# lucas-t-t/FACT-CLIP

Hardware: AMD Instinct MI355X
Metric: frames/sec FACT_CLIP fwd+bwd, T=4096 D=2048 Nact=32, at 1/2/4/8 GPUs (higher is better)
Workload: dtype fp32; 1 GPU; FACT_CLIP HAViD-holdout dims, seg10 synthetic, T=4096; model=FACT_CLIP, T=4096, D=2048, Nact=32, C=75, videos_per_rank=2, global_batch=2, seq_len=4096, parallelism=dp1, weights=fixed (no optimizer update in the timed steps)

## Files before the change

fact-clip_amd/csrc/capi.cpp:

```cpp
#include <algorithm>
#include <atomic>
#include <tuple>
#include <map>
#include <mutex>
#include <cmath>
#include <cstdlib>
#include <cstring>
#include <mutex>
#include <vector>

#include "fx_common.h"
#include "ops.h"

namespace fx {

static thread_local std::string g_last_error;
void set_error(const std::string& msg) { g_last_error = msg; }

namespace {
struct ProfState {
  int max_events = 0;
  std::vector<hipEvent_t> ev;
  std::vector<double> flops, bytes;
  std::vector<int> launches;
// ... 414 lines not shown
  long long d = p->dil0 > 0 ? p->dil0 : 1;
  const int f = p->dil_factor > 0 ? p->dil_factor : 2;
  for (int k = 0; k < i; ++k) d *= f;
  return (int)d;
}

bool mstcn_defer_ok(const fx_mstcn_params* p, const fx_mstcn_grads* g) {
  if (!knobs().mstcn_defer) return false;
  const int NL = p->num_layers;
  for (int i = 0; i < NL; ++i)
    if (!g->w_dil[i] || !g->b_dil[i] || !g->w_pw[i] || !g->b_pw[i]) return false;
  auto uniform = [&](float* const* v) {
    for (int i = 2; i < NL; ++i)
      if (v[i] - v[i - 1] != v[1] - v[0]) return false;
    return true;
  };
  return uniform(g->w_dil) && uniform(g->b_dil) && uniform(g->w_pw) && uniform(g->b_pw);
}

struct Seqs {
  int T, nvid;
  const int* off;
  int rows() const { return off ? off[nvid] : T * nvid; }
  int start(int v) const { return off ? off[v] : v * T; }
  int len(int v) const { return off ? off[v + 1] - off[v] : T; }
};

int check_seqs(const Seqs& q) {
  FX_REQUIRE(q.nvid >= 1, "frame branch: nvid >= 1");
  if (!q.off) {
    FX_REQUIRE(q.T >= 1, "frame branch: T >= 1");
    return FX_OK;
  }
  FX_REQUIRE(q.nvid <= 16 && q.off[0] == 0, "frame branch: ragged offsets start at 0, <= 16 videos");
  for (int v = 0; v < q.nvid; ++v) FX_REQUIRE(q.off[v + 1] > q.off[v], "frame branch: empty video");
  return FX_OK;
}

fx_operand conv_operand(const float* h, long long ld, int cin, int dil, int dir, const Seqs& q, bool trans) {
  fx_operand o = trans ? op_cols(h, ld) : op_rows(h, ld);
  o.conv_taps = 3;
  o.conv_cin = cin;
  o.conv_dil = dil;
  o.conv_dir = dir;
  if (q.off) {
    o.seq_off = q.off;
    o.nseq = q.nvid;
  } else {
    o.seq_len = q.T;
  }
  return o;
}

template <typename Fn>
int per_video(const Seqs& q, Fn fn) {
  if (!q.off) return fn(0, q.rows(), q);
  for (int v = 0; v < q.nvid; ++v) FX_TRY(fn(q.start(v), q.len(v), Seqs{q.len(v), 1, nullptr}));
  return FX_OK;
}

}
}

using namespace fx;

extern "C" {

int fx_version(void) { return FX_ABI_VERSION; }

}

namespace fx {
const Knobs& knobs() {
  static Knobs k;
  static std::once_flag once;
  std::call_once(once, [] {
    auto env = [](const char* n) -> const char* { return std::getenv(n); };
    if (const char* p = env("FX_GEMM_PATH")) k.gemm_path = std::string(p) == "tiled" ? 1 : std::string(p) == "direct" ? 2 : 0;
    if (const char* p = env("FX_GEMM_W8")) k.gemm_w8 = p[0] == '1';
    if (const char* p = env("FX_GEMM_WIDE")) k.gemm_wide = p[0] == '1' ? 1 : 0;
    if (const char* p = env("FX_GEMM_XCDPLANES")) k.gemm_xcd_planes = p[0] != '0';
    if (const char* p = env("FX_GEMM_GROUP")) k.gemm_group = p[0] != '0';
    if (const char* p = env("FX_GEMM_KTAIL")) k.gemm_ktail = p[0] != '0';
    if (const char* p = env("FX_DEC_TOK")) k.dec_tok = p[0] != '0';
    if (const char* p = env("FX_TOK_SPIN")) k.tok_spin = std::max(0, std::atoi(p));
    if (const char* p = env("FX_SIDE_STREAM")) k.side_stream = p[0] != '0';
    if (const char* p = env("FX_MSTCN_DEFER")) k.mstcn_defer = p[0] != '0';
    if (const char* p = env("FX_GEMM_ROWPERM")) k.gemm_row_perm = p[0] != '0';
    if (const char* p = env("FX_GEMM_GROUPM")) k.gemm_group_m = p[0] != '0';
    if (const char* p = env("FX_GEMM_PERSIST")) k.gemm_persist = p[0] != '0';
    if (const char* p = env("FX_FRL_XCD")) k.frl_xcd = std::atoi(p);
    if (const char* p = env("FX_FRL_PAIR")) k.frl_pair = p[0] != '0';
    if (const char* p = env("FX_FRL_MIN_FILL")) k.frl_min_fill = std::atoi(p);
    if (const char* p = env("FX_AUX_STREAM")) k.aux_stream = p[0] != '0';
    if (const char* p = env("FX_GRU_POLL2")) k.gru_poll2 = p[0] != '0';
    if (const char* p = env("FX_GRU_STORE_WAVE")) k.gru_store_wave = std::max(0, std::min(2, std::atoi(p)));
    if (const char* p = env("FX_TATTN_RR")) k.tattn_rr = p[0] != '0';
    if (const char* p = env("FX_X2Y_A2F_DW")) k.x2y_a2f_dw = p[0] != '0';
    if (const char* p = env("FX_TATTN_FOLD")) k.tattn_fold = p[0] != '0';
    if (const char* p = env("FX_X2Y_FUSED")) k.x2y_fused = p[0] != '0';
    if (const char* p = env("FX_X2Y_F2A_BWD")) k.x2y_f2a_bwd = std::atoi(p);
    if (const char* p = env("FX_X2Y_F2A_ONE")) k.x2y_f2a_one = p[0] != '0';
  });
  return k;
}
}

extern "C" {
const char* fx_last_error(void) { return g_last_error.c_str(); }

int fx_dropout(const float* x, long long ldx, int rows, int cols, long long idx_ld, long long idx_col0, float p,
               unsigned long long seed, float* y, long long ldy, void* stream) {
  FX_REQUIRE(x && y && rows >= 0 && cols >= 0, "dropout: bad arguments");
  return launch_dropout(x, ldx, rows, cols, idx_ld, idx_col0, p, seed, y, ldy, (hipStream_t)stream);
}

long long fx_struct_size(int which) {
  switch (which) {
    case 0: return (long long)sizeof(fx_gemm_desc);
    case 1: return (long long)sizeof(fx_decoder_params);
    case 2: return (long long)sizeof(fx_mstcn_params);
    case 3: return (long long)sizeof(fx_loss_term);
    case 4: return (long long)sizeof(fx_video_attn);
    case 5: return (long long)sizeof(fx_mstcn2_params);
    default: return -1;
  }
}

int fx_gemm(const fx_gemm_desc* desc, void* stream) {
  FX_REQUIRE(desc, "fx_gemm: null descriptor");
  const bool conv = desc->a.conv_taps && !desc->a.trans;
  if (conv) prof_begin(0, (hipStream_t)stream);
  const int st = launch_gemm(*desc, (hipStream_t)stream);
  if (conv) prof_end(0, (hipStream_t)stream, 2.0 * desc->M * desc->N * desc->K * desc->batch, 0.0);
  return st;
}

long long fx_gemm_workspace_floats(const fx_gemm_desc* desc) { return desc ? gemm_workspace_floats(*desc) : 0; }

int fx_linear_fwd(const float* x, long long ldx, const float* pos, long long ldpos, int pos_cols, int M, int K,
                  const float* w, long long ldw, const float* b, float* y, long long ldy, int N, int relu,
                  void* stream) {
  return linear_fwd(x, ldx, M, K, w, b, y, ldy, N, relu, (hipStream_t)stream, ldw, pos, ldpos, pos_cols);
}

long long fx_linear_bwd_workspace_floats(int M, int K, int N) {
  return (long long)M * N + split_ws(M, K, N) + dwdb_ws(M, K, N) + colsum_workspace_floats(M, N);
}

int fx_linear_bwd(const float* dy, long long lddy, const float* x, long long ldx, const float* w, long long ldw,
                  const float* relu_out, long long ld_relu, int M, int K, int N, float* dx, long long lddx,
                  float* dw, long long lddw, float* db, int accumulate_dx, int accumulate_w, float* workspace,
                  void* stream) {
  hipStream_t s = (hipStream_t)stream;
  FX_REQUIRE(workspace || (!relu_out && split_ws(M, K, N) == 0 && dwdb_ws(M, K, N) == 0 && !(db && !dw)),
             "fx_linear_bwd: workspace required");
  float* wz = workspace;
  float* wsx = wz + (long long)M * N;
  float* wsw = wsx + split_ws(M, K, N);
  float* wsc = wsw + dwdb_ws(M, K, N);
  const float* g = dy;
  long long ldg = lddy;
  if (relu_out) {
    FX_TRY(relu_bwd(dy, lddy, relu_out, ld_relu, M, N, wz, N, s));
    g = wz;
    ldg = N;
// ... 1490 lines not shown
```

fact-clip_amd/csrc/fx_common.h:

```cpp
#pragma once
#include <hip/hip_runtime.h>
#include <hip/hip_ext.h>
#include <cstdint>
#include <cstdio>
#include <string>

#include "../../include/factmx.h"

namespace fx {

void set_error(const std::string& msg);

#define FX_CHECK_HIP(expr)                                                        \
  do {                                                                            \
    hipError_t _e = (expr);                                                       \
    if (_e != hipSuccess) {                                                       \
      ::fx::set_error(std::string("HIP error ") + hipGetErrorString(_e) + " at " + \
                      __FILE__ + ":" + std::to_string(__LINE__));                 \
      return FX_ERR_HIP;                                                          \
    }                                                                             \
  } while (0)

#define FX_REQUIRE(cond, msg)                 \
  do {                                        \
    if (!(cond)) {                            \
      ::fx::set_error(std::string(msg));      \
      return FX_ERR_SHAPE;                    \
    }                                         \
  } while (0)

#define FX_TRY(expr)                 \
  do {                               \
    int _s = (expr);                 \
    if (_s != FX_OK) return _s;      \
  } while (0)

inline int cdiv(long long a, long long b) { return (int)((a + b - 1) / b); }
inline long long al64(long long n) { return (n + 63) & ~63LL; }

int launch_gemm(const fx_gemm_desc& d, hipStream_t s);
int launch_gemm_group(const fx_gemm_desc* d, int n, hipStream_t s);

struct WsBound {
  WsBound(const float* base, long long floats);
  ~WsBound();
  const float* prev_lo;
  const float* prev_hi;
};
hipStream_t side_fork(hipStream_t s, int event);
int side_join_into(hipStream_t s);
hipStream_t aux_fork(hipStream_t s);
int aux_join_into(hipStream_t s, hipStream_t a);
int defer_split(int rows);
long long gemm_workspace_floats(const fx_gemm_desc& d);

fx_operand op_rows(const float* p, long long ld);
fx_operand op_cols(const float* p, long long ld);
fx_gemm_desc gemm_desc(int M, int N, int K, fx_operand a, fx_operand b, float* c, long long ldc);

int launch_colsum_batched(const float* x, long long ld, long long x_bs, int M, int N, int nb, float* out,
                          long long out_bs, int accumulate, float* ws, hipStream_t s);
int launch_colsum(const float* x, long long ld, int M, int N, float* out, int accumulate,
                  float* ws, hipStream_t s);

constexpr long long kArrivalCounters = 1 << 16;
unsigned* arrival_counters(hipStream_t s);

__host__ __device__ inline unsigned fx_drop_bits(unsigned long long seed, unsigned long long idx) {
  unsigned long long z = seed + (idx + 1ull) * 0x9E3779B97F4A7C15ull;
  z = (z ^ (z >> 30)) * 0xBF58476D1CE4E5B9ull;
  z = (z ^ (z >> 27)) * 0x94D049BB133111EBull;
  z ^= z >> 31;
  return (unsigned)(z >> 32);
}
inline unsigned fx_drop_thresh(float p) {
  const double t = (double)p * 4294967296.0;
  return t >= 4294967295.0 ? 4294967295u : (unsigned)t;
}
inline unsigned long long fx_drop_subseed(unsigned long long seed, int i) {
  return seed + 0xD1B54A32D192ED03ull * (unsigned long long)(i + 1);
}
int launch_dropout(const float* x, long long ldx, int rows, int cols, long long idx_ld, long long idx_col0, float p,
                   unsigned long long seed, float* y, long long ldy, hipStream_t s);

struct Knobs {
  int gemm_path = 0;
  bool gemm_w8 = true;
  int gemm_wide = -1;
  bool gemm_xcd_planes = true;
  bool gemm_persist = true;
  bool gemm_group_m = true;
  bool gemm_row_perm = true;
  bool frl_pair = true;
  int frl_min_fill = 80;
  bool aux_stream = true;
  bool x2y_a2f_dw = true;
  bool tattn_fold = true;
  bool tattn_rr = true;
  bool gru_poll2 = true;
  int gru_store_wave = 2;
  int frl_xcd = 2;
  bool gemm_group = true;
  bool gemm_ktail = true;
  bool dec_tok = true;
  int tok_spin = 0;
  bool side_stream = true;
  bool mstcn_defer = true;
  bool x2y_fused = true;
  bool x2y_f2a_one = true;
  int x2y_f2a_bwd = 2;
};
const Knobs& knobs();

void prof_begin(int kind, hipStream_t s);
void prof_end(int kind, hipStream_t s, double flops, double bytes, int launches = 1);
extern thread_local int g_prof_open;
bool prof_kernel_events(hipStream_t s, hipEvent_t* e0, hipEvent_t* e1);

template <typename... Args, typename F = void (*)(Args...)>
inline void fx_launch(F kernel, const dim3& grid, const dim3& block, std::uint32_t shm, hipStream_t s, Args... args) {
  hipEvent_t e0, e1;
  if (g_prof_open >= 0 && prof_kernel_events(s, &e0, &e1))
    hipExtLaunchKernelGGL(kernel, grid, block, shm, s, e0, e1, 0u, args...);
  else
    hipLaunchKernelGGL(kernel, grid, block, shm, s, args...);
}

unsigned tok_spin_max();
unsigned x2y_spin_max();
int coresident_blocks(const void* kernel, int threads, size_t lds);

}
```

fact-clip_amd/csrc/gemm_f32.hip:

```cpp
#include <algorithm>
#include <atomic>
#include <cstdio>
#include <cstdlib>
#include <map>
#include <mutex>
#include <string>
#include <utility>
#include <vector>

#include "fx_common.h"

namespace fx {
namespace {

constexpr int BM = 64, BN = 64, BK = 64, NTHREADS = 256;
constexpr int RS = 68;
constexpr int CS = 65;
constexpr int IMG = BM * RS;
constexpr int NSLOT = 3;
typedef float f32x16 __attribute__((ext_vector_type(16)));

constexpr int kMaxSeq = 16;

enum Kind { ROWS = 0, ROWS_CONV = 1, ROWS_GEN = 2, COLS = 3, COLS_CONV = 4, ROWS_CAT = 5, COLS_CONVR = 6, COLS_KT = 7 };
// ... 1617 lines not shown
      if constexpr (AK == COLS_KT) {
        if (!fast) break;
        fx_launch((gemm_f32_kernel<AK, COLS_KT, true>), grid, dim3(NTHREADS), 0, s, g);
        return FX_OK;
      }
      break;
    case ROWS_GEN:
    case ROWS_CAT: launch_t<AK, ROWS_GEN>(grid, s, g, false); return FX_OK;
    default: break;
  }
  set_error("gemm: unsupported B operand kind");
  return FX_ERR_UNSUPPORTED;
}

int launch_tiled(int ak, int bk, dim3 grid, hipStream_t s, const GemmDev& g) {
  const bool fast = g.a_vec && g.b_vec && ((g.K % BK) == 0 || ak == COLS_KT) && ak != ROWS_GEN && bk != ROWS_GEN;
  switch (ak) {
    case ROWS: return launch_b<ROWS>(bk, grid, s, g, fast);
    case ROWS_CONV: return launch_b<ROWS_CONV>(bk, grid, s, g, fast);
    case ROWS_GEN: return launch_b<ROWS_GEN>(bk, grid, s, g, false);
    case ROWS_CAT: return launch_b<ROWS_CAT>(bk, grid, s, g, fast);
    case COLS: return launch_b<COLS>(bk, grid, s, g, fast);
    case COLS_KT: return launch_b<COLS_KT>(bk, grid, s, g, fast);
    default: break;
  }
  set_error("gemm: unsupported A operand kind");
  return FX_ERR_UNSUPPORTED;
}

template <int AK>
int launch_direct_b(int bk, dim3 grid, dim3 block, hipStream_t s, const GemmDev& g) {
  switch (bk) {
    case ROWS: fx_launch((gemm_direct_kernel<AK, ROWS>), grid, block, 0, s, g); return FX_OK;
    case COLS: fx_launch((gemm_direct_kernel<AK, COLS>), grid, block, 0, s, g); return FX_OK;
    default: break;
  }
  set_error("gemm(direct): unsupported B operand kind");
  return FX_ERR_UNSUPPORTED;
}

int launch_direct(int ak, int bk, dim3 grid, dim3 block, hipStream_t s, const GemmDev& g) {
  switch (ak) {
    case ROWS: return launch_direct_b<ROWS>(bk, grid, block, s, g);
    case ROWS_GEN:
    case ROWS_CAT: return launch_direct_b<ROWS_GEN>(bk, grid, block, s, g);
    case COLS: return launch_direct_b<COLS>(bk, grid, block, s, g);
    default: break;
  }
  set_error("gemm(direct): unsupported A operand kind");
  return FX_ERR_UNSUPPORTED;
}

bool use_direct(const fx_gemm_desc& d, int ak, int bk) {
  const int force = knobs().gemm_path;
  auto fits = [&](const fx_operand& o, int kind, int R) {
    const double k = (double)d.K + 2 * DMAXW * DCH + 64, ld = (double)o.ld;
    const double bytes = kind == ROWS ? ((double)R * ld + k) * 4 : kind == COLS ? (k * ld + R) * 4 : 0;
    return bytes < 4294967296.0;
  };
  const bool ok = d.K > 0 && (ak == ROWS || ak == ROWS_GEN || ak == ROWS_CAT || ak == COLS) && (bk == ROWS || bk == COLS) &&
                  fits(d.a, ak, d.M) && fits(d.b, bk, d.N);
  if (!ok || force == 1) return false;
  if (force == 2) return true;
  const int lim = (ak == ROWS_GEN || ak == ROWS_CAT) ? 32 : 64;
  if (d.M <= lim || d.N <= lim || d.K <= 64 || (d.K <= 512 && d.K % 64 != 0)) return true;
  const long long t32 = (long long)cdiv(d.M, 32) * cdiv(d.N, 32) * d.batch;
  return (ak == ROWS || ak == COLS) && t32 <= 512 && d.K <= 2048;
}

bool wide8() {
  return knobs().gemm_w8;
}

bool use_wide(const GemmDev& g, int ak, int bk, int batch) {
  const int force = knobs().gemm_wide;
  const bool fast = g.a_vec && g.b_vec && ((g.K % BK) == 0 || ak == COLS_KT);
  const bool ok = fast && (ak == ROWS || ak == ROWS_CONV || ak == ROWS_CAT || ak == COLS || ak == COLS_KT) &&
                  (bk == ROWS || bk == COLS || bk == COLS_CONV || bk == COLS_CONVR || bk == COLS_KT);
  if (!ok || force == 0) return false;
  if (force == 1) return true;
  return (long long)cdiv(g.M, WBM) * g.tiles_x * batch * g.split >= 192;
}

constexpr long long kMaxTileCounters = kArrivalCounters;
unsigned* tile_counters(hipStream_t s) {
  static std::mutex mu;
  static std::map<std::pair<int, hipStream_t>, unsigned*> pool;
  int dev = 0;
  if (hipGetDevice(&dev) != hipSuccess) return nullptr;
  std::lock_guard<std::mutex> lk(mu);
  const auto key = std::make_pair(dev, s);
  auto it = pool.find(key);
  if (it != pool.end()) return it->second;
  unsigned* p = nullptr;
  if (hipMalloc(&p, kMaxTileCounters * sizeof(unsigned)) != hipSuccess) return nullptr;
  if (hipMemsetAsync(p, 0, kMaxTileCounters * sizeof(unsigned), s) != hipSuccess) {
    (void)hipFree(p);
    return nullptr;
  }
  pool[key] = p;
  return p;
}

}

unsigned* arrival_counters(hipStream_t s) { return tile_counters(s); }


thread_local const float* t_ws_lo = nullptr;
thread_local const float* t_ws_hi = nullptr;

WsBound::WsBound(const float* base, long long floats) : prev_lo(t_ws_lo), prev_hi(t_ws_hi) {
  t_ws_lo = base;
  t_ws_hi = base ? base + std::max(floats, 0LL) : nullptr;
}
WsBound::~WsBound() {
  t_ws_lo = prev_lo;
  t_ws_hi = prev_hi;
}

fx_operand op_rows(const float* p, long long ld) {
  fx_operand o{};
  o.ptr = p;
  o.ld = ld;
  o.conv_dir = 1;
  return o;
}

fx_operand op_cols(const float* p, long long ld) {
  fx_operand o = op_rows(p, ld);
  o.trans = 1;
  return o;
}

fx_gemm_desc gemm_desc(int M, int N, int K, fx_operand a, fx_operand b, float* c, long long ldc) {
  fx_gemm_desc d{};
  d.M = M;
  d.N = N;
  d.K = K;
  d.batch = 1;
  d.a = a;
  d.b = b;
  d.c = c;
  d.ldc = ldc;
  d.alpha = 1.f;
  d.split_k = 1;
  return d;
}

long long gemm_workspace_floats(const fx_gemm_desc& d) {
  if (d.split_k <= 1) return 0;
  return (long long)d.batch * d.split_k * d.M * d.N;
}

namespace {

struct GemmPlan {
  GemmDev g;
  dim3 grid, block;
  int ak, bk;
  bool direct, wide;
};

int plan_gemm(const fx_gemm_desc& d, hipStream_t s, GemmPlan& P, long long tile_cnt_base = 0) {
  FX_REQUIRE(d.M >= 0 && d.N >= 0 && d.K >= 0 && d.batch >= 1, "gemm: bad sizes");
  FX_REQUIRE(d.a.ptr && d.b.ptr && d.c, "gemm: null operand");
  FX_REQUIRE(!(d.a.conv_taps && d.a.seq_len <= 0 && d.a.nseq <= 0) &&
                 !(d.b.conv_taps && d.b.seq_len <= 0 && d.b.nseq <= 0),
             "gemm: conv operand needs seq_len or seq_off");
  FX_REQUIRE(d.a.nseq <= 0 || !d.a.trans, "gemm: ragged conv offsets on a row-major A or a column-major B operand");
  FX_REQUIRE(d.b.nseq <= 0 || (d.b.trans && d.b.conv_taps && d.a.nseq <= 0),
             "gemm: ragged column-major conv B needs a plain A operand");
  FX_REQUIRE(!(d.a.conv_taps && d.K != d.a.conv_taps * d.a.conv_cin), "gemm: conv A needs K == taps*cin");
  FX_REQUIRE(!(d.b.conv_taps && d.b.trans && d.N != d.b.conv_taps * d.b.conv_cin + (d.b.ones_col ? 1 : 0)),
             "gemm: conv B needs N == taps*cin (+1 with a ones column)");
  FX_REQUIRE(!(d.a.ones_col && !d.a.trans) && !(d.b.ones_col && !d.b.trans), "gemm: ones_col needs trans==1");
  FX_REQUIRE(!(d.b.conv_taps && !d.b.trans), "gemm: row-major conv B operand is not supported");
  GemmDev& g = P.g;
  g = GemmDev{};
  g.M = d.M;
  g.N = d.N;
  g.K = d.K;
  g.a = d.a;
  g.b = d.b;
  {
    const fx_operand& o = d.a;
    if (o.nseq > 0) {
      FX_REQUIRE(o.conv_taps && o.seq_off && o.nseq <= kMaxSeq, "gemm: seq_off needs a conv operand, <= 16 videos");
      const int rows = d.M;
      FX_REQUIRE(o.seq_off[0] == 0 && o.seq_off[o.nseq] == rows, "gemm: seq_off must span the operand's rows");
      for (int v = 0; v <= o.nseq; ++v) {
        FX_REQUIRE(v == 0 || o.seq_off[v] > o.seq_off[v - 1], "gemm: seq_off must increase");
        g.soff[v] = o.seq_off[v];
      }
      g.nsoff = o.nseq;
    }
  }
  {
    const fx_operand& o = d.b;
    if (o.nseq > 0) {
      FX_REQUIRE(o.seq_off && o.nseq <= kMaxSeq && o.seq_off[0] == 0 && o.seq_off[o.nseq] <= d.K,
                 "gemm: ragged B offsets must start at 0 and end within K, <= 16 videos");
      FX_REQUIRE(operand_vec_ok(d.a) && operand_vec_ok(d.b) && d.K % BK == 0,
                 "gemm: ragged B needs 16-B operands and K a multiple of 64 (pad the frames)");
      for (int v = 0; v <= kMaxSeq; ++v) {
        FX_REQUIRE(v == 0 || v > o.nseq || o.seq_off[v] > o.seq_off[v - 1], "gemm: seq_off must increase");
        g.soff[v] = v <= o.nseq ? o.seq_off[v] : 0x7fffffff;
      }
      g.nsoff = o.nseq;
    }
  }
  g.c = d.c;
  g.ldc = d.ldc;
  g.c_bs = d.c_batch_stride;
  g.alpha = d.alpha;
  g.beta = d.beta;
  g.bias = d.bias;
  g.resid = d.resid;
  g.ld_resid = d.ld_resid;
  g.resid_bs = d.resid_batch_stride;
  g.gate = d.gate;
  g.ld_gate = d.ld_gate;
  g.relu = d.relu;
  g.c_tap_cin = d.c_tap_cin;
  g.c_last = d.c_last_col;
  g.c_last_bs = d.c_last_batch_stride ? d.c_last_batch_stride : d.M;
  g.b_dil_growth = d.b_dil_growth;
  g.a_dil_b1 = d.a_dil_b1;
  g.bias_bs = d.bias_batch_stride;
  FX_REQUIRE(d.a_dil_b1 <= 0 || (d.a.conv_taps && !d.a.trans), "gemm: a_dil_b1 needs a row-major conv A");
  FX_REQUIRE(d.b_dil_growth <= 1 || (d.b.conv_taps && d.b.trans), "gemm: b_dil_growth needs a column-major conv B");
  g.stamps = d.dbg_stamps;
  FX_REQUIRE(d.drop_p >= 0.f && d.drop_p < 1.f, "gemm: dropout p must be in [0, 1)");
  FX_REQUIRE(d.drop_p == 0.f || (!d.c_last_col && !d.c_tap_cin && !d.gate && d.beta == 0.f &&
                                 !(d.relu == 1 && d.resid)),
             "gemm: dropout only on plain outputs (before the residual add)");
  g.drop_thr = d.drop_p > 0.f ? std::max(fx_drop_thresh(d.drop_p), 1u) : 0u;
  g.drop_scale = 1.f / (1.f - d.drop_p);
  g.drop_seed = d.drop_seed;
  g.a_vec = operand_vec_ok(d.a);
  g.b_vec = operand_vec_ok(d.b);
  g.ws = d.workspace;
  int ak = kind_of(d.a, g.a_vec), bk = kind_of(d.b, g.b_vec);
  const bool direct = d.b_dil_growth <= 1 && d.a_dil_b1 <= 0 && use_direct(d, ak, bk);
  if (!direct && ak == COLS && bk == COLS && g.a_vec && g.b_vec && d.K % BK != 0 && knobs().gemm_ktail) ak = bk = COLS_KT;
  P.ak = ak;
  P.bk = bk;
  bool wide = false;
  const int cap = (d.split_k > 1 && d.workspace) ? d.split_k : 1;
  FX_REQUIRE(!(d.split_k > 1 && !d.workspace), "gemm: split-K needs a workspace");
  dim3 grid, block;
  if (direct) {
    const int nch = cdiv(d.K, DCH);
    const long long t32 = (long long)cdiv(d.M, 32) * cdiv(d.N, 32) * d.batch;
    const int cpw = 1;
    const int nw = std::min(DMAXW, std::max(1, nch / cpw));
    int split = 1;
    if (cap > 1 && t32 < 64) {
      const long long want = std::min<long long>(nch / (cpw * nw), cdiv(2048, t32 * nw));
      split = (int)std::max<long long>(1, std::min<long long>(cap, want));
    }
    g.kt_per_split = nch > 0 ? cdiv(nch, split) : 0;
    g.split = g.kt_per_split > 0 ? cdiv(nch, g.kt_per_split) : 1;
    g.tiles_x = cdiv(d.N, 32);
    g.tiles_y = cdiv(d.M, 32);
    grid = dim3(g.tiles_x, g.tiles_y, d.batch * g.split);
    block = dim3(nw * 64);
  } else {
    const int nkt = cdiv(d.K, BK);
    int split = std::min(cap, std::max(nkt, 1));
    g.kt_per_split = nkt > 0 ? cdiv(nkt, split) : 0;
    g.split = g.kt_per_split > 0 ? cdiv(nkt, g.kt_per_split) : 1;
    g.tiles_x = cdiv(d.N, BN);
    wide = use_wide(g, ak, bk, d.batch);
    g.tiles_y = cdiv(d.M, wide ? WBM : BM);
    grid = dim3(g.tiles_x, g.tiles_y, d.batch * g.split);
    block = dim3(NTHREADS);
  }
  if (g.split > 1 && t_ws_hi && !(g.ws >= t_ws_lo && g.ws + (long long)g.split * d.M * d.N * d.batch <= t_ws_hi))
    std::fprintf(stderr, "factmx: gemm M %d N %d K %d batch %d split %d (cap %d, %s) needs %lld floats at +%lld of a %lld-float reservation\n",
                 d.M, d.N, d.K, d.batch, g.split, cap, direct ? "direct" : "tiled",
                 (long long)g.split * d.M * d.N * d.batch, (long long)(g.ws - t_ws_lo), (long long)(t_ws_hi - t_ws_lo));
  FX_REQUIRE(g.split <= 1 || !t_ws_hi ||
                 (g.ws >= t_ws_lo && g.ws + (long long)g.split * d.M * d.N * d.batch <= t_ws_hi),
             "gemm: split-K slabs would overrun the entry point's workspace reservation");
  const long long slab_bytes = (long long)g.split * (direct ? 32 * 32 : (wide ? WBM : BM) * BN) * 4;
  if (g.split > 1 && slab_bytes <= 32768 &&
      tile_cnt_base + (long long)g.tiles_x * g.tiles_y * d.batch <= kMaxTileCounters) {
    unsigned* pool = tile_counters(s);
    g.tile_cnt = pool ? pool + tile_cnt_base : nullptr;
  }
  const bool planes_on = knobs().gemm_xcd_planes;
  const long long nz = (long long)d.batch * g.split;
  g.xcd_planes = planes_on && wide && wide8() && nz >= 8 && nz % 8 == 0;
  if (knobs().gemm_row_perm && wide && !g.xcd_planes && d.a.conv_taps > 1 && !d.a.trans && d.a_dil_b1 <= 0) {
    const int sh = d.a.conv_dil / WBM;
    if (sh > 1 && g.tiles_y % sh == 0) g.row_perm = sh;
  }
  g.group_m = 0;
  if (knobs().gemm_group_m && !g.xcd_planes && g.row_perm <= 1 && d.a.conv_taps <= 1 && d.b.conv_taps <= 1 &&
      g.tiles_y >= 16 && g.tiles_x >= 8) {
    const int gm = g.tiles_y / 8, tm = wide ? WBM : BM;
    const double b_bytes = 4.0 * d.N * d.K, a_run = 4.0 * gm * tm * d.K;
    if (b_bytes > 2.0 * (1 << 20) && a_run <= 2.0 * (1 << 20)) g.group_m = gm;
  }
  g.persist = 0;
  P.grid = grid;
  P.block = block;
  P.direct = direct;
  P.wide = wide;
  return FX_OK;
}

int launch_reduce(const fx_gemm_desc& d, const GemmPlan& P, hipStream_t s) {
  if (P.g.split > 1 && !P.g.tile_cnt) {
    const long long total = (long long)d.M * d.N;
    const int vec = (total % 4) == 0 && ((uintptr_t)P.g.ws & 15) == 0;
    int blocks = (int)std::min<long long>(cdiv(cdiv(total, 4), 256), 2048);
    fx_launch(splitk_reduce_kernel, dim3(blocks, d.batch), dim3(256), 0, s, P.g, vec);
    FX_CHECK_HIP(hipGetLastError());
  }
  return FX_OK;
}

}

std::mutex g_prec_mu;
std::vector<std::pair<hipStream_t, int>> g_prec;
std::atomic<int> g_prec_any{0};
std::atomic<int> g_prec_default{FX_PREC_F32};
// ... 2 lines not shown
  if (!g_prec_any.load(std::memory_order_acquire)) return g_prec_default.load(std::memory_order_relaxed);
  std::lock_guard<std::mutex> lk(g_prec_mu);
  for (const auto& e : g_prec)
    if (e.first == s) return e.second;
  return g_prec_default.load(std::memory_order_relaxed);
}

bool valid_precision(int prec) {
  return prec == FX_PREC_F32 || prec == FX_PREC_BF16 || prec == FX_PREC_F32S || prec == FX_PREC_F32S2;
}

bool rowmajor_wide(const GemmPlan& P) {
  return P.wide && (P.bk == ROWS || P.bk == COLS) && (P.ak == ROWS || P.ak == ROWS_CONV || P.ak == ROWS_CAT);
}
bool bf16_eligible(const GemmPlan& P, hipStream_t s) {
  return rowmajor_wide(P) && stream_precision(s) == FX_PREC_BF16;
}
int split_pieces_for(const GemmPlan& P, hipStream_t s) {
  if (!rowmajor_wide(P)) return 0;
  const int prec = stream_precision(s);
  return prec == FX_PREC_F32S ? 3 : prec == FX_PREC_F32S2 ? 2 : 0;
}

template <int AK, int NP>
int launch_split_b(const GemmPlan& P, hipStream_t s) {
  if (P.bk == ROWS)
    fx_launch((gemm_f32_wide8_kernel<AK, ROWS, NP>), P.grid, dim3(W8T), 0, s, P.g);
  else
    fx_launch((gemm_split_wide8_kernel<AK, COLS, NP>), P.grid, dim3(W8T), 0, s, P.g);
  return FX_OK;
}

template <int NP>
int launch_split_np(const GemmPlan& P, hipStream_t s) {
  switch (P.ak) {
    case ROWS: return launch_split_b<ROWS, NP>(P, s);
    case ROWS_CONV: return launch_split_b<ROWS_CONV, NP>(P, s);
    case ROWS_CAT: return launch_split_b<ROWS_CAT, NP>(P, s);
    default: break;
  }
  set_error("gemm(split): unsupported A operand kind");
  return FX_ERR_UNSUPPORTED;
}

int launch_split(const GemmPlan& P, int np, hipStream_t s) {
  return np == 3 ? launch_split_np<3>(P, s) : launch_split_np<2>(P, s);
}

template <int AK>
int launch_bf16_b(const GemmPlan& P, hipStream_t s) {
  if (P.bk == ROWS)
    fx_launch((gemm_bf16_wide8_kernel<AK, ROWS>), P.grid, dim3(W8T), 0, s, P.g);
  else
    fx_launch((gemm_bf16_wide8_kernel<AK, COLS>), P.grid, dim3(W8T), 0, s, P.g);
  return FX_OK;
}

int launch_bf16(const GemmPlan& P, hipStream_t s) {
  switch (P.ak) {
    case ROWS: return launch_bf16_b<ROWS>(P, s);
    case ROWS_CONV: return launch_bf16_b<ROWS_CONV>(P, s);
    case ROWS_CAT: return launch_bf16_b<ROWS_CAT>(P, s);
    default: break;
  }
  set_error("gemm(bf16): unsupported A operand kind");
  return FX_ERR_UNSUPPORTED;
}

int launch_gemm(const fx_gemm_desc& d, hipStream_t s) {
  FX_REQUIRE(d.M >= 0 && d.N >= 0 && d.K >= 0 && d.batch >= 1, "gemm: bad sizes");
  if (d.M == 0 || d.N == 0) return FX_OK;
  GemmPlan P;
  FX_TRY(plan_gemm(d, s, P));
  const int np = split_pieces_for(P, s);
  if (knobs().gemm_persist && !np && !bf16_eligible(P, s) && P.wide && wide8() && P.g.split == 1 && d.batch == 1 &&
      !P.g.xcd_planes) {
    const long long nt = (long long)P.g.tiles_x * P.g.tiles_y;
    constexpr int G = 256;
    if (nt >= 2 * G) {
      P.g.persist = (int)nt;
      P.grid = dim3(G, 1, 1);
    }
  }
  const GemmDev& g = P.g;
#ifdef FX_GEMM_CENSUS
  std::fprintf(stderr, "GEMM %p %d %d %d %d %d %d %d %d %d %d %d\n", (void*)s, d.M, d.N, d.K, d.batch, P.ak, P.bk,
               P.g.split, P.direct ? 1 : P.wide ? 2 : 0, P.g.persist, d.a.conv_taps, (int)(P.g.split > 1 && !P.g.tile_cnt));
#endif
  int st = np ? launch_split(P, np, s)
         : bf16_eligible(P, s) ? launch_bf16(P, s)
         : P.direct ? launch_direct(P.ak, P.bk, P.grid, P.block, s, g)
                    : (P.wide ? (wide8() ? launch_wide8(P.ak, P.bk, P.grid, s, g) : launch_wide(P.ak, P.bk, P.grid, s, g))
                              : launch_tiled(P.ak, P.bk, P.grid, s, g));
  if (st != FX_OK) return st;
  FX_CHECK_HIP(hipGetLastError());
  return launch_reduce(d, P, s);
}

int launch_gemm_group(const fx_gemm_desc* d, int n, hipStream_t s) {
  const bool on = knobs().gemm_group;
  FX_REQUIRE(n >= 0 && n <= GMAX, "gemm group: 0..4 members");
  int live = 0, nsplit = 0;
  bool all_direct = on;
  GemmPlan P[GMAX];
  long long cnt_base = 0;
  for (int i = 0; i < n && all_direct; ++i) {
    FX_REQUIRE(d[i].M >= 0 && d[i].N >= 0 && d[i].K >= 0 && d[i].batch >= 1, "gemm: bad sizes");
    if (d[i].M == 0 || d[i].N == 0) continue;
    FX_TRY(plan_gemm(d[i], s, P[i], cnt_base));
    if (P[i].g.tile_cnt) cnt_base += (long long)P[i].g.tiles_x * P[i].g.tiles_y * d[i].batch;
    all_direct = all_direct && P[i].direct;
    nsplit += P[i].g.split > 1 ? 1 : 0;
    ++live;
  }
  bool ws_ok = true;
  if (all_direct && nsplit > 1) {
    const float* base = nullptr;
    long long off = 0;
    for (int i = 0; i < n && ws_ok; ++i) {
      if (d[i].M == 0 || d[i].N == 0 || P[i].g.split <= 1) continue;
      if (!base) base = d[i].workspace;
      ws_ok = d[i].workspace == base && t_ws_hi != nullptr;
      P[i].g.ws = d[i].workspace + off;
      off += (long long)P[i].g.split * d[i].M * d[i].N * d[i].batch;
      ws_ok = ws_ok && P[i].g.ws >= t_ws_lo && P[i].g.ws + (long long)P[i].g.split * d[i].M * d[i].N * d[i].batch <= t_ws_hi;
    }
  }
  if (!all_direct || live < 2 || !ws_ok) {
    for (int i = 0; i < n; ++i) FX_TRY(launch_gemm(d[i], s));
    return FX_OK;
  }
  bool done[GMAX] = {};
  for (int i0 = 0; i0 < n; ++i0) {
    if (done[i0] || d[i0].M == 0 || d[i0].N == 0) continue;
    const unsigned nw = P[i0].block.x;
    GemmGroup G{};
    int m = 0;
    G.start[0] = 0;
    for (int i = i0; i < n; ++i) {
      if (done[i] || d[i].M == 0 || d[i].N == 0 || P[i].block.x != nw) continue;
      done[i] = true;
      G.g[m] = P[i].g;
      const int ak = P[i].ak == ROWS_CAT ? ROWS_GEN : P[i].ak;
      G.kinds[m] = ak * 8 + P[i].bk;
      G.start[m + 1] = G.start[m] + (int)(P[i].grid.x * P[i].grid.y * P[i].grid.z);
      ++m;
    }
    for (int i = m + 1; i <= GMAX; ++i) G.start[i] = G.start[m];
    G.n = m;
    if (m == 1) {
#ifdef FX_GEMM_CENSUS
      std::fprintf(stderr, "GEMM %p %d %d %d %d %d %d %d 1 0 0 %d\n", (void*)s, d[i0].M, d[i0].N, d[i0].K, d[i0].batch,
                   P[i0].ak, P[i0].bk, P[i0].g.split, (int)(P[i0].g.split > 1 && !P[i0].g.tile_cnt));
#endif
      FX_TRY(P[i0].direct ? launch_direct(P[i0].ak, P[i0].bk, P[i0].grid, P[i0].block, s, P[i0].g) : FX_ERR_UNSUPPORTED);
    } else {
      fx_launch(gemm_direct_group_kernel, dim3(G.start[m]), dim3(nw), 0, s, G);
    }
    FX_CHECK_HIP(hipGetLastError());
  }
  for (int i = 0; i < n; ++i)
    if (d[i].M != 0 && d[i].N != 0) FX_TRY(launch_reduce(d[i], P[i], s));
  return FX_OK;
}

int launch_colsum_batched(const float* x, long long ld, long long x_bs, int M, int N, int nb, float* out,
                          long long out_bs, int accumulate, float* ws, hipStream_t s) {
  if (N == 0 || nb == 0) return FX_OK;
  if (M == 0) {
    if (!accumulate)
      for (int b = 0; b < nb; ++b) FX_CHECK_HIP(hipMemsetAsync(out + (long long)b * out_bs, 0, sizeof(float) * N, s));
    return FX_OK;
  }
  const int nblk = cdiv(M, CS_ROWS);
  fx_launch(colsum_stage1, dim3(cdiv(N, 64), nblk, nb), dim3(256), 0, s, x, ld, x_bs, M, N, ws);
  fx_launch(colsum_stage2, dim3(cdiv(N, 256), nb), dim3(256), 0, s, ws, nblk, N, out, out_bs, accumulate);
  FX_CHECK_HIP(hipGetLastError());
  return FX_OK;
}

int launch_colsum(const float* x, long long ld, int M, int N, float* out, int accumulate, float* ws,
                  hipStream_t s) {
  return launch_colsum_batched(x, ld, 0, M, N, 1, out, 0, accumulate, ws, s);
}

long long colsum_workspace_floats(int M, int N) { return (long long)cdiv(M, CS_ROWS) * N; }

}

extern "C" {

int fx_set_stream_precision(void* stream, int prec) {
  FX_REQUIRE(prec == FX_PREC_DEFAULT || fx::valid_precision(prec),
             "gemm precision: FX_PREC_DEFAULT, FX_PREC_F32, FX_PREC_BF16, FX_PREC_F32S or FX_PREC_F32S2");
// ... 32 lines not shown
```

Before: 585,700 frames/s.

## Add persistent stream-K MFMA kernel for weight-gradient GEMMs

Adds a dedicated persistent kernel for transposed-A by transposed-B (weight-gradient) GEMMs. It uses 128x128x32 tiles with a three-slot LDS pipeline and fp32 MFMA 32x32x2. K-iterations are split evenly across a resident-sized grid in stream-K fashion, with partials written to workspace and fixed up by the last arriving block through tile counters. It also fuses the ones-column bias-gradient row sum into the same pass. The aim is to balance long-K reductions across CUs instead of using split-K plus a separate reduce launch. The cost is atomic fixup traffic and an extra planning path that the group launcher must now avoid.

```diff
diff --git a/fact-clip_amd/csrc/capi.cpp b/fact-clip_amd/csrc/capi.cpp
--- a/fact-clip_amd/csrc/capi.cpp
+++ b/fact-clip_amd/csrc/capi.cpp
@@ -520,6 +520,9 @@
     if (const char* p = env("FX_GEMM_XCDPLANES")) k.gemm_xcd_planes = p[0] != '0';
     if (const char* p = env("FX_GEMM_GROUP")) k.gemm_group = p[0] != '0';
     if (const char* p = env("FX_GEMM_KTAIL")) k.gemm_ktail = p[0] != '0';
+    if (const char* p = env("FX_GEMM_DW")) k.gemm_dw = p[0] == '0' ? 0 : p[0] == '1' ? 1 : -1;
+    if (const char* p = env("FX_GEMM_DW_OVERSUB")) k.gemm_dw_oversub = std::max(1, std::atoi(p));
+    if (const char* p = env("FX_GEMM_DW_GRID")) k.gemm_dw_grid = std::max(0, std::atoi(p));
     if (const char* p = env("FX_DEC_TOK")) k.dec_tok = p[0] != '0';
     if (const char* p = env("FX_TOK_SPIN")) k.tok_spin = std::max(0, std::atoi(p));
     if (const char* p = env("FX_SIDE_STREAM")) k.side_stream = p[0] != '0';
diff --git a/fact-clip_amd/csrc/fx_common.h b/fact-clip_amd/csrc/fx_common.h
--- a/fact-clip_amd/csrc/fx_common.h
+++ b/fact-clip_amd/csrc/fx_common.h
@@ -101,6 +101,9 @@
   int gru_store_wave = 2;
   int frl_xcd = 2;
   bool gemm_group = true;
+  int gemm_dw = -1;
+  int gemm_dw_oversub = 1;
+  int gemm_dw_grid = 0;
   bool gemm_ktail = true;
   bool dec_tok = true;
   int tok_spin = 0;
diff --git a/fact-clip_amd/csrc/gemm_f32.hip b/fact-clip_amd/csrc/gemm_f32.hip
--- a/fact-clip_amd/csrc/gemm_f32.hip
+++ b/fact-clip_amd/csrc/gemm_f32.hip
@@ -1723,6 +1723,299 @@
   return (long long)cdiv(g.M, WBM) * g.tiles_x * batch * g.split >= 192;
 }
 
+constexpr int DWM = 128, DWN = 128, DWK = 32, DWT = 256;
+constexpr int DWA = DWK * DWM;
+constexpr int DWSLOT = DWK * (DWM + DWN);
+constexpr int DWPART = DWM * DWN + 2 * DWT;
+constexpr int DWLDS = 38 * 1024;
+typedef float f32x2 __attribute__((ext_vector_type(2)));
+
+struct DwPlan {
+  int S;
+  int T;
+  long long U;
+  int aligned;
+  int bias;
+  int G;
+  int np, nb, mem;
+};
+
+__device__ __forceinline__ int dw_workgroup(const DwPlan& p) {
+  const int per = gridDim.x >> 3;
+  const int pos = (blockIdx.x & 7) * per + (blockIdx.x >> 3);
+  if (pos >= p.G) return -1;
+  const int group = pos / p.mem, member = pos - group * p.mem;
+  const int plane = group / p.nb, r = group - plane * p.nb;
+  return plane * p.np + r + p.nb * member;
+}
+
+__device__ __forceinline__ long long dw_run_start(const DwPlan& p, int w, int G) {
+  return p.aligned ? ((long long)w * p.T / G) * p.S : (long long)w * p.U / G;
+}
+__device__ __forceinline__ int dw_owner(const DwPlan& p, long long u, int G) {
+  return (int)(((u + 1) * G - 1) / p.U);
+}
+
+template <int BKd>
+struct DwLoader {
+  const float* pa;
+  const float* pb;
+  long long lda, ldb;
+  int lk, lr;
+  int seq_len, tap_s;
+
+  __device__ __forceinline__ void init(const GemmDev& g, int bidx, int m0, int n0, int tid) {
+    lk = tid >> 5;
+    lr = (tid & 31) * 4;
+    lda = g.a.ld;
+    ldb = g.b.ld;
+    const int ra = min(m0 + lr, ((g.M - 1) / 4) * 4);
+    pa = g.a.ptr + (long long)bidx * g.a.batch_stride + (long long)lk * lda + ra;
+    const int rb = min(n0 + lr, ((g.N - 1) / 4) * 4);
+    const float* b0 = g.b.ptr + (long long)bidx * g.b.batch_stride;
+    if (BKd == COLS_CONV) {
+      const fx_operand ob = batch_op_b(g.b, g.b_dil_growth, bidx);
+      const int j = rb / ob.conv_cin;
+      tap_s = conv_shift(ob, j);
+      seq_len = ob.seq_len;
+      pb = b0 + (rb - j * ob.conv_cin);
+    } else {
+      tap_s = 0;
+      seq_len = 1;
+      pb = b0 + (long long)lk * ldb + rb;
+    }
+  }
+  __device__ __forceinline__ void load_a(int s, float4* v) const {
+#pragma unroll
+    for (int j = 0; j < 4; ++j) v[j] = ldg4(pa + (long long)(s * DWK + 8 * j) * lda);
+  }
+  __device__ __forceinline__ void load_b(int s, float4* v, unsigned& vm) const {
+    if (BKd == COLS_CONV) {
+      vm = 0;
+#pragma unroll
+      for (int j = 0; j < 4; ++j) {
+        const int k = s * DWK + lk + 8 * j;
+        const int t = k % seq_len + tap_s;
+        const bool ok = t >= 0 && t < seq_len;
+        vm |= (ok ? 1u : 0u) << j;
+        v[j] = ldg4(pb + (long long)(ok ? k + tap_s : k) * ldb);
+      }
+    } else {
+      vm = 0xFu;
+#pragma unroll
+      for (int j = 0; j < 4; ++j) v[j] = ldg4(pb + (long long)(s * DWK + 8 * j) * ldb);
+    }
+  }
+  __device__ __forceinline__ void store_a(float* slot, const float4* v) const {
+#pragma unroll
+    for (int j = 0; j < 4; ++j) *reinterpret_cast<float4*>(slot + (lk + 8 * j) * DWM + lr) = v[j];
+  }
+  __device__ __forceinline__ void store_b(float* slot, const float4* v, unsigned vm) const {
+#pragma unroll
+    for (int j = 0; j < 4; ++j) {
+      const float4 x = (BKd != COLS_CONV || ((vm >> j) & 1u)) ? v[j] : zero4();
+      *reinterpret_cast<float4*>(slot + DWA + (lk + 8 * j) * DWN + lr) = x;
+    }
+  }
+};
+
+template <int BKd>
+__device__ __forceinline__ void dw_stage(const DwLoader<BKd>& L, const float* cur, float* wslot, int sload,
+                                         const float4* sa, const float4* sb, unsigned sm, float4* na, float4* nb,
+                                         unsigned& nm, int offa, int offb, f32x16& c00, f32x16& c01, f32x16& c10,
+                                         f32x16& c11, float& rs0, float& rs1, const float* nxt, f32x2* ca, f32x2* cb) {
+  const float* ia = cur + offa;
+  const float* ib = cur + DWA + offb;
+  f32x2 fa[DWK / 2], fb[DWK / 2];
+  fa[0] = ca[0];
+  fb[0] = cb[0];
+  fa[1] = ca[1];
+  fb[1] = cb[1];
+  __builtin_amdgcn_sched_barrier(0);
+#pragma unroll
+  for (int q = 0; q < DWK / 2; ++q) {
+    c00 = __builtin_amdgcn_mfma_f32_32x32x2f32(fa[q].x, fb[q].x, c00, 0, 0, 0);
+    c01 = __builtin_amdgcn_mfma_f32_32x32x2f32(fa[q].x, fb[q].y, c01, 0, 0, 0);
+    c10 = __builtin_amdgcn_mfma_f32_32x32x2f32(fa[q].y, fb[q].x, c10, 0, 0, 0);
+    c11 = __builtin_amdgcn_mfma_f32_32x32x2f32(fa[q].y, fb[q].y, c11, 0, 0, 0);
+    rs0 += fa[q].x;
+    rs1 += fa[q].y;
+    if (q + 2 < DWK / 2) {
+      fa[q + 2] = *reinterpret_cast<const f32x2*>(ia + (q + 2) * 2 * DWM);
+      fb[q + 2] = *reinterpret_cast<const f32x2*>(ib + (q + 2) * 2 * DWN);
+    }
+    if (q == 0) L.load_a(sload, na);
+    if (q == 1) L.load_b(sload, nb, nm);
+    if (q == 11) L.store_a(wslot, sa);
+    if (q == 13) L.store_b(wslot, sb, sm);
+    if (q == DWK / 2 - 2) {
+      ca[0] = *reinterpret_cast<const f32x2*>(nxt + offa);
+      cb[0] = *reinterpret_cast<const f32x2*>(nxt + DWA + offb);
+      ca[1] = *reinterpret_cast<const f32x2*>(nxt + offa + 2 * DWM);
+      cb[1] = *reinterpret_cast<const f32x2*>(nxt + DWA + offb + 2 * DWN);
+    }
+    __builtin_amdgcn_sched_barrier(0);
+  }
+}
+
+template <int BKd>
+__device__ __forceinline__ void dw_kloop(const DwLoader<BKd>& L, float* lds, int s0, int s1, int offa, int offb,
+                                         f32x16& c00, f32x16& c01, f32x16& c10, f32x16& c11, float& rs0, float& rs1) {
+  const int n = s1 - s0, slast = s1 - 1;
+  float4 ax[4], bx[4], ay[4], by[4];
+  unsigned mx, my;
+  L.load_a(s0, ax);
+  L.load_b(s0, bx, mx);
+  L.load_a(min(s0 + 1, slast), ay);
+  L.load_b(min(s0 + 1, slast), by, my);
+  L.store_a(lds, ax);
+  L.store_b(lds, bx, mx);
+  L.store_a(lds + DWSLOT, ay);
+  L.store_b(lds + DWSLOT, by, my);
+  L.load_a(min(s0 + 2, slast), ax);
+  L.load_b(min(s0 + 2, slast), bx, mx);
+  __syncthreads();
+  f32x2 ca[2], cb[2];
+  ca[0] = *reinterpret_cast<const f32x2*>(lds + offa);
+  cb[0] = *reinterpret_cast<const f32x2*>(lds + DWA + offb);
+  ca[1] = *reinterpret_cast<const f32x2*>(lds + offa + 2 * DWM);
+  cb[1] = *reinterpret_cast<const f32x2*>(lds + DWA + offb + 2 * DWN);
+  int slot = 0;
+  auto iter = [&](int i, const float4* sa, const float4* sb, unsigned sm, float4* na, float4* nb, unsigned& nm) FX_INLINE {
+    const int ws = slot == 0 ? 2 : slot - 1, ns = slot == 2 ? 0 : slot + 1;
+    dw_stage<BKd>(L, lds + slot * DWSLOT, lds + ws * DWSLOT, min(s0 + i + 3, slast), sa, sb, sm, na, nb, nm, offa, offb,
+                  c00, c01, c10, c11, rs0, rs1, lds + ns * DWSLOT, ca, cb);
+    __syncthreads();
+    slot = ns;
+  };
+  int i = 0;
+  for (; i + 1 < n; i += 2) {
+    iter(i, ax, bx, mx, ay, by, my);
+    iter(i + 1, ay, by, my, ax, bx, mx);
+  }
+  if (i < n) iter(i, ax, bx, mx, ay, by, my);
+}
+
+__device__ __forceinline__ void dw_store_block(const GemmDev& g, float* cb, int rbase, int col, const f32x16& acc) {
+  if (col >= g.N) return;
+  long long cc = col;
+  if (g.c_tap_cin) {
+    const int j = col / g.c_tap_cin;
+    cc = (long long)(col - j * g.c_tap_cin) * 3 + j;
+  }
+  float* p = cb + cc;
+  float cold[16];
+#pragma unroll
+  for (int r = 0; r < 16; ++r) {
+    const int row = min(rbase + 2 * ((r & 3) + 8 * (r >> 2)), g.M - 1);
+    cold[r] = g.beta != 0.f ? p[(long long)row * g.ldc] : 0.f;
+  }
+#pragma unroll
+  for (int r = 0; r < 16; ++r) {
+    const int row = rbase + 2 * ((r & 3) + 8 * (r >> 2));
+    float v = g.alpha * acc[r];
+    if (g.beta != 0.f) v += g.beta * cold[r];
+    if (row < g.M) p[(long long)row * g.ldc] = v;
+  }
+}
+
+template <int BKd>
+__global__ __launch_bounds__(DWT) void gemm_dw_kernel(GemmDev g, DwPlan p) {
+  __shared__ float lds[DWLDS];
+  const int tid = threadIdx.x, lane = tid & 63, wave = tid >> 6;
+  const int wm = wave >> 1, wn = wave & 1, li = lane & 31, lh = lane >> 5;
+  const int offa = lh * DWM + wm * 64 + 2 * li, offb = lh * DWN + wn * 64 + 2 * li;
+  const int w = dw_workgroup(p), G = p.G;
+  if (w < 0) return;
+  int* flag = reinterpret_cast<int*>(&lds[DWLDS - 1]);
+  const long long ubeg = dw_run_start(p, w, G), uend = dw_run_start(p, w + 1, G);
+  const int tfirst = (int)(ubeg / p.S);
+  for (long long u = ubeg; u < uend;) {
+    const int t = (int)(u / p.S);
+    const int s0 = (int)(u - (long long)t * p.S);
+    const int s1 = (int)min((long long)p.S, s0 + (uend - u));
+    u += s1 - s0;
+    const int tx = t % g.tiles_x, ty = (t / g.tiles_x) % g.tiles_y, bidx = t / (g.tiles_x * g.tiles_y);
+    const int m0 = ty * DWM, n0 = tx * DWN;
+    DwLoader<BKd> L;
+    L.init(g, bidx, m0, n0, tid);
+    f32x16 c00, c01, c10, c11;
+#pragma unroll
+    for (int i = 0; i < 16; ++i) c00[i] = c01[i] = c10[i] = c11[i] = 0.f;
+    float rs0 = 0.f, rs1 = 0.f;
+    dw_kloop<BKd>(L, lds, s0, s1, offa, offb, c00, c01, c10, c11, rs0, rs1);
+    if (s1 - s0 < p.S) {
+      float* part = g.ws + (long long)(2 * w + (t == tfirst ? 0 : 1)) * DWPART;
+      float4* p4 = reinterpret_cast<float4*>(part);
+#pragma unroll
+      for (int r = 0; r < 4; ++r) {
+        p4[(0 + r) * DWT + tid] = make_float4(c00[4 * r], c00[4 * r + 1], c00[4 * r + 2], c00[4 * r + 3]);
+        p4[(4 + r) * DWT + tid] = make_float4(c01[4 * r], c01[4 * r + 1], c01[4 * r + 2], c01[4 * r + 3]);
+        p4[(8 + r) * DWT + tid] = make_float4(c10[4 * r], c10[4 * r + 1], c10[4 * r + 2], c10[4 * r + 3]);
+        p4[(12 + r) * DWT + tid] = make_float4(c11[4 * r], c11[4 * r + 1], c11[4 * r + 2], c11[4 * r + 3]);
+      }
+      reinterpret_cast<f32x2*>(part + DWM * DWN)[tid] = f32x2{rs0, rs1};
+      const int wa = dw_owner(p, (long long)t * p.S, G), wb = dw_owner(p, (long long)t * p.S + p.S - 1, G);
+      asm volatile("s_waitcnt vmcnt(0)" ::: "memory");
+      __syncthreads();
+      if (tid == 0) {
+        __builtin_amdgcn_fence(__ATOMIC_RELEASE, "agent");
+        asm volatile("s_waitcnt vmcnt(0)" ::: "memory");
+        const unsigned prev = __hip_atomic_fetch_add(&g.tile_cnt[t], 1u, __ATOMIC_RELAXED, __HIP_MEMORY_SCOPE_AGENT);
+        const int last = prev == (unsigned)(wb - wa);
+        if (last) {
+          __hip_atomic_store(&g.tile_cnt[t], 0u, __ATOMIC_RELAXED, __HIP_MEMORY_SCOPE_AGENT);
+          __builtin_amdgcn_fence(__ATOMIC_ACQUIRE, "agent");
+          asm volatile("s_waitcnt vmcnt(0)" ::: "memory");
+        }
+        *flag = last;
+      }
+      __syncthreads();
+      const int last = *flag;
+      __syncthreads();
+      if (!last) continue;
+#pragma unroll
+      for (int i = 0; i < 16; ++i) c00[i] = c01[i] = c10[i] = c11[i] = 0.f;
+      rs0 = rs1 = 0.f;
+      for (int c = wa; c <= wb; ++c) {
+        const int cfirst = (int)(dw_run_start(p, c, G) / p.S);
+        const float* cp = g.ws + (long long)(2 * c + (t == cfirst ? 0 : 1)) * DWPART;
+        const float4* c4 = reinterpret_cast<const float4*>(cp);
+        float4 v[16];
+#pragma unroll
+        for (int r = 0; r < 16; ++r) v[r] = c4[r * DWT + tid];
+        const f32x2 rs = reinterpret_cast<const f32x2*>(cp + DWM * DWN)[tid];
+#pragma unroll
+        for (int r = 0; r < 4; ++r) {
+          c00[4 * r] += v[r].x; c00[4 * r + 1] += v[r].y; c00[4 * r + 2] += v[r].z; c00[4 * r + 3] += v[r].w;
+          c01[4 * r] += v[4 + r].x; c01[4 * r + 1] += v[4 + r].y; c01[4 * r + 2] += v[4 + r].z; c01[4 * r + 3] += v[4 + r].w;
+          c10[4 * r] += v[8 + r].x; c10[4 * r + 1] += v[8 + r].y; c10[4 * r + 2] += v[8 + r].z; c10[4 * r + 3] += v[8 + r].w;
+          c11[4 * r] += v[12 + r].x; c11[4 * r + 1] += v[12 + r].y; c11[4 * r + 2] += v[12 + r].z; c11[4 * r + 3] += v[12 + r].w;
+        }
+        rs0 += rs.x;
+        rs1 += rs.y;
+      }
+    } else {
+      __syncthreads();
+    }
+    float* cb = g.c + (long long)bidx * g.c_bs;
+    const int rbase = m0 + wm * 64 + 8 * lh, col = n0 + wn * 64 + 2 * li;
+    dw_store_block(g, cb, rbase, col, c00);
+    dw_store_block(g, cb, rbase, col + 1, c01);
+    dw_store_block(g, cb, rbase + 1, col, c10);
+    dw_store_block(g, cb, rbase + 1, col + 1, c11);
+    if (p.bias && tx == 0 && wn == 0) {
+      const float t0 = rs0 + __shfl_xor(rs0, 32), t1 = rs1 + __shfl_xor(rs1, 32);
+      const int row = m0 + wm * 64 + 2 * li;
+      float* bp = g.c_last + (long long)bidx * g.c_last_bs;
+      if (lh == 0) {
+        if (row < g.M) bp[row] = g.alpha * t0 + (g.beta != 0.f ? g.beta * bp[row] : 0.f);
+        if (row + 1 < g.M) bp[row + 1] = g.alpha * t1 + (g.beta != 0.f ? g.beta * bp[row + 1] : 0.f);
+      }
+    }
+  }
+}
+
 constexpr long long kMaxTileCounters = kArrivalCounters;
 unsigned* tile_counters(hipStream_t s) {
   static std::mutex mu;
@@ -1801,7 +2094,77 @@
   dim3 grid, block;
   int ak, bk;
   bool direct, wide;
+  bool dw;
+  DwPlan dwp;
 };
+
+const char* plan_dw(const fx_gemm_desc& d, hipStream_t s, GemmPlan& P, bool direct, long long tile_cnt_base) {
+  GemmDev& g = P.g;
+  const bool force = knobs().gemm_dw == 1;
+  if (P.ak != COLS || (P.bk != COLS && P.bk != COLS_CONV)) return "operand kinds other than COLS x COLS / COLS_CONV";
+  if (!g.a_vec || !g.b_vec || d.K % BK != 0) return "operands not 16-B aligned or K not a multiple of 64";
+  if (d.K < 2 * BK) return "K below two 64-deep stages";
+  if (d.M < DWM) return "M below one 128-row tile";
+  if (d.bias || d.resid || d.gate || d.relu || d.drop_p > 0.f || d.a_dil_b1 > 0) return "epilogue other than alpha / beta / c_tap_cin / c_last";
+  if (d.a.ones_col) return "ones column on A";
+  const bool ones = d.b.ones_col != 0;
+  if (ones && (d.b.ones_col != d.N || !d.c_last_col)) return "ones column that is not B's last column routed to c_last";
+  if (!ones && d.c_last_col) return "c_last without a ones column";
+  const int N = d.N - (ones ? 1 : 0);
+  if (N < 1) return "no stored column";
+  const int tx = cdiv(N, DWN), ty = cdiv(d.M, DWM);
+  const long long T = (long long)tx * ty * d.batch;
+  const int S = d.K / DWK;
+  if (T * S > 0x7fffffffLL || tile_cnt_base + T > kMaxTileCounters) return "too many tiles";
+  const void* kern = P.bk == COLS ? (const void*)gemm_dw_kernel<COLS> : (const void*)gemm_dw_kernel<COLS_CONV>;
+  const int resident = coresident_blocks(kern, DWT, 0);
+  if (resident < 1) return "kernel cannot be resident";
+  long long ws_floats = (d.split_k > 1 && d.workspace && aligned16(d.workspace)) ? gemm_workspace_floats(d) : 0;
+  if (ws_floats && t_ws_hi)
+    ws_floats = (g.ws >= t_ws_lo && g.ws <= t_ws_hi) ? std::min<long long>(ws_floats, t_ws_hi - g.ws) : 0;
+  const long long gp = ws_floats / (2 * DWPART);
+  unsigned* pool = gp >= 2 ? tile_counters(s) : nullptr;
+  DwPlan& p = P.dwp;
+  p.S = S;
+  p.T = (int)T;
+  p.U = T * S;
+  p.aligned = (pool && gp >= d.batch) ? 0 : 1;
+  p.bias = ones ? 1 : 0;
+  long long G;
+  if (p.aligned) {
+    G = std::min<long long>(resident, T);
+    p.np = p.mem = (int)G;
+    p.nb = 1;
+  } else {
+    const long long tpp = (long long)tx * ty;
+    long long slots = (long long)resident * std::max(1, knobs().gemm_dw_oversub);
+    if (knobs().gemm_dw_grid > 0) slots = std::min<long long>(slots, knobs().gemm_dw_grid);
+    long long np = std::min<long long>(std::min<long long>(slots, gp) / d.batch, tpp * S);
+    auto gcd = [](long long a, long long b) { while (b) { const long long t = a % b; a = b; b = t; } return a; };
+    while (np > 1 && np / gcd(np, tpp) > 8) --np;
+    p.np = (int)np;
+    p.nb = (int)(np / gcd(np, tpp));
+    p.mem = p.np / p.nb;
+    G = np * d.batch;
+  }
+  p.G = (int)G;
+  if (!force) {
+    if (direct) return "the direct kernel's shape";
+    if (d.K < 2048 || T < 32 || G < 128) return "too few tiles or too short a K for the persistent grid";
+  }
+  g.N = N;
+  g.tiles_x = tx;
+  g.tiles_y = ty;
+  g.split = 1;
+  g.kt_per_split = 0;
+  g.tile_cnt = pool ? pool + tile_cnt_base : nullptr;
+  P.grid = dim3((unsigned)(cdiv(G, 8) * 8));
+  P.block = dim3(DWT);
+  P.direct = false;
+  P.wide = false;
+  P.dw = true;
+  return nullptr;
+}
 
 int plan_gemm(const fx_gemm_desc& d, hipStream_t s, GemmPlan& P, long long tile_cnt_base = 0) {
   FX_REQUIRE(d.M >= 0 && d.N >= 0 && d.K >= 0 && d.batch >= 1, "gemm: bad sizes");
@@ -1887,6 +2250,15 @@
   if (!direct && ak == COLS && bk == COLS && g.a_vec && g.b_vec && d.K % BK != 0 && knobs().gemm_ktail) ak = bk = COLS_KT;
   P.ak = ak;
   P.bk = bk;
+  P.dw = false;
+  if (d.a.trans && d.b.trans && knobs().gemm_dw != 0) {
+    const char* why = plan_dw(d, s, P, direct, tile_cnt_base);
+    if (!why) return FX_OK;
+    if (knobs().gemm_dw == 1) {
+      set_error(std::string("gemm(dw): FX_GEMM_DW=1 but the planner cannot route this product: ") + why);
+      return FX_ERR_UNSUPPORTED;
+    }
+  }
   bool wide = false;
   const int cap = (d.split_k > 1 && d.workspace) ? d.split_k : 1;
   FX_REQUIRE(!(d.split_k > 1 && !d.workspace), "gemm: split-K needs a workspace");
@@ -2055,6 +2427,14 @@
       P.grid = dim3(G, 1, 1);
     }
   }
+  if (P.dw) {
+    if (P.bk == COLS)
+      fx_launch(gemm_dw_kernel<COLS>, P.grid, P.block, 0, s, P.g, P.dwp);
+    else
+      fx_launch(gemm_dw_kernel<COLS_CONV>, P.grid, P.block, 0, s, P.g, P.dwp);
+    FX_CHECK_HIP(hipGetLastError());
+    return FX_OK;
+  }
   const GemmDev& g = P.g;
 #ifdef FX_GEMM_CENSUS
   std::fprintf(stderr, "GEMM %p %d %d %d %d %d %d %d %d %d %d %d\n", (void*)s, d.M, d.N, d.K, d.batch, P.ak, P.bk,
@@ -2082,7 +2462,7 @@
     if (d[i].M == 0 || d[i].N == 0) continue;
     FX_TRY(plan_gemm(d[i], s, P[i], cnt_base));
     if (P[i].g.tile_cnt) cnt_base += (long long)P[i].g.tiles_x * P[i].g.tiles_y * d[i].batch;
-    all_direct = all_direct && P[i].direct;
+    all_direct = all_direct && P[i].direct && !P[i].dw;
     nsplit += P[i].g.split > 1 ? 1 : 0;
     ++live;
   }
```

Measured after the change: 583,000 frames/s. About the same (-0.5%).
